# byteowlz/kokorox

Hardware: AMD Instinct MI355X
Metric: real-time factor (audio-s/wall-s), 24 kHz, batch=64 (higher is better)
Workload: dtype f32 in / out, f32 accumulate; products on split operands: f16f8 (a_hi b_hi on f16 MFMAs, the cross terms a_lo b_hi + a_hi b_lo of the 7 / 11-tap convs on e4m3 scaled MFMAs: ~17 significant bits per product; every other conv f16x3: ~22) -- wider than the bf16 BASELINE configs[2] names, inside the 1e-; 1 GPU; batch=64/GPU synthetic 128-phoneme utterances (T=130), durations pinned 3,3,3,4 -> F=422 frames = 10.55 s each, noise on, inputs in HBM; batch_per_gpu=64, frames=422, parallelism=utterance-sharded x1, one-time weight broadcast

## Files before the change

kokorox_amd/build.py:

```python
from __future__ import annotations

import os
import subprocess
import sys

HERE = os.path.dirname(os.path.abspath(__file__))
CSRC = os.path.join(HERE, "csrc")
LIB_DIR = os.path.join(HERE, "lib")
LIB_PATH = os.path.join(LIB_DIR, "libkokorox_hip.so")
TEST_LIB_PATH = os.path.join(LIB_DIR, "libkokorox_hip_test.so")
TEST_SOURCES = ["test_hooks.hip"]
SOURCES = ["conv_plan.hip", "conv_call.hip", "conv_mfma.hip", "conv_f16x3.hip", "conv_f16x3_da.hip", "conv_f16x3_da_p1.hip", "conv_f16x3_da_w2.hip", "conv_f16x3_da_s16.hip", "conv_f16x3_da_f8.hip", "conv_f16x3_da_pre.hip", "conv_f16x3_pre.hip", "conv_f16x3_dapn.hip", "conv_f16x3_dag.hip", "kernels_misc.hip", "model.hip", "model_forward.hip", "model_host.hip", "api.hip", "dispatcher.hip", "onnx_import.cpp", "kxw_file.cpp",
           "host_request.cpp", "host_pool.cpp"]
HEADERS = ["kx_common.h", "kx_error.h", "host_request.h", "conv_epilogue.h", "conv_f16x3_common.h"]
_PUB = os.path.join("..", "..", "include", "kokorox_hip.h")
_PUB_TEST = os.path.join("..", "..", "include", "kokorox_hip_test.h")
_MODEL_H = ["model.h", "kxw_file.h", "onnx_import.h"]
EXTRA_DEPS = {"model.hip": [*_MODEL_H, _PUB], "model_forward.hip": [*_MODEL_H, _PUB], "model_host.hip": [*_MODEL_H, "host_pool.h", _PUB],
              "host_pool.cpp": ["host_pool.h"], "host_request.cpp": ["resample_taps.h"], "kernels_misc.hip": ["resample_taps.h"], "conv_call.hip": _MODEL_H, "api.hip": [*_MODEL_H, "kx_handle.h", "api_guard.h", "check_device.h", _PUB],
              "dispatcher.hip": [*_MODEL_H, "kx_handle.h", "dispatcher_core.h", _PUB],
              "test_hooks.hip": [*_MODEL_H, "kx_handle.h", "api_guard.h", "check_device.h", _PUB, _PUB_TEST], "onnx_import.cpp": ["onnx_import.h"],
              "kxw_file.cpp": ["kxw_file.h", "onnx_import.h"], "conv_f16x3_da_p1.hip": ["conv_f16x3_da.hip"], "conv_f16x3_da_w2.hip": ["conv_f16x3_da.hip"], "conv_f16x3_da_s16.hip": ["conv_f16x3_da.hip"], "conv_f16x3_da_f8.hip": ["conv_f16x3_da.hip"], "conv_f16x3_da_pre.hip": ["conv_f16x3_da.hip"]}
FLAGS = ["-O3", "--offload-arch=gfx950", "-fPIC", "-std=c++17", "-Wall", "-Wno-unused-result"]


def _hipcc() -> str:
    for cand in (os.environ.get("HIPCC"), "/opt/rocm/bin/hipcc", "hipcc"):
        if cand and (os.path.isabs(cand) and os.path.exists(cand) or not os.path.isabs(cand)):
            return cand
    return "hipcc"


def _newer(target: str, deps) -> bool:
    if not os.path.exists(target):
        return False
    t = os.path.getmtime(target)
    return all(os.path.getmtime(d) <= t for d in deps)


LAST_BUILD = {"compiled": [], "reused": [], "linked": False}


def build_library(force: bool = False, verbose: bool = False) -> str:
    LAST_BUILD["compiled"], LAST_BUILD["reused"], LAST_BUILD["linked"] = [], [], False
    os.makedirs(LIB_DIR, exist_ok=True)
# ... 40 lines not shown
```

kokorox_amd/csrc/conv_f16x3.hip:

```cpp
#include "conv_f16x3_common.h"

namespace kx {

template <int BM, int BN, int WM, int WN, int ACT, int TK, bool PF, int VT>
__global__ __launch_bounds__(WM * WN * 64, (WM * WN == 8) ? 4 : ((BM / WM / 32) * (BN / WN / 32) > 6 ? 2 : 3))
void conv1d_f16x3_kernel(const ConvArgs a) {
    constexpr int MT = BM / WM / 32;
    constexpr int NT = BN / WN / 32;
    constexpr int NWV = WM * WN;
    static_assert((NWV == 4 || NWV == 8) && MT >= 1 && NT >= 1, "4 or 8 waves per workgroup");
    static_assert(VT == 1 || (VT <= TK && PF), "virtual taps need TK >= VT and the prefetching build");
    extern __shared__ __attribute__((aligned(16))) unsigned char smem16[];

    const int tid = threadIdx.x;
    const int lane = tid & 63;
    const int wave = __builtin_amdgcn_readfirstlane(tid >> 6);
    const int wm = wave / WN, wn = wave % WN;
    const int r = lane & 31, h = lane >> 5;
    const int b = blockIdx.z, ct = blockIdx.y;
    int tile_x = blockIdx.x;
    if (a.xcd_swizzle && gridDim.x >= 16) {
        const int nx = gridDim.x;
        const int off = (int)(((long)nx * (blockIdx.y + (long)gridDim.y * blockIdx.z)) & 7);
        const int cls = (blockIdx.x + off) & 7;
// ... 364 lines not shown
    else if (bm == 32 && bn == 256 && wm == 1 && wn == 4)
        launch_inst16<32, 256, 1, 4>(p, a, B, s);
    else
        throw Error(1, "conv1d f16x3: no such LDS-DMA form");
}

void launch_conv(const ConvPlan& p, const ConvArgs& a, int B, hipStream_t s) {
    if (p.form == FORM_F32) {
        launch_conv1d(a, p.bm, B, p.cols, s);
        return;
    }
    KX_REQUIRE(a.n_chunks16 == (a.Cin + CK16 - 1) / CK16 && a.w16 != nullptr, "conv1d f16x3: weights not packed");
    KX_REQUIRE(a.epi != EPI_GELU_NEW || p.vt > 1 || p.form == FORM_DAG || p.form == FORM_DAGN,
               "conv1d f16x3: gelu epilogue exists only for k=1 GEMMs with >= 48 input channels");
    KX_REQUIRE(p.merged == (a.merge_T > 0), "conv1d f16x3: merged columns do not match the plan");
    if (p.cols <= 0) return;
    switch (p.form) {
        case FORM_LDS: launch_lds(p, a, B, s); return;
        case FORM_DAG:
        case FORM_DAGN: launch_conv1d_f16x3_dag(p, a, B, s); return;
        case FORM_DAPN: launch_conv1d_f16x3_dapn(a, B, p.cols, s); return;
        case FORM_DA_PRE: launch_conv16_da_pre(p, a, B, s); return;
        case FORM_DA_S16: launch_conv16_da_s16(p, a, B, s); return;
        case FORM_DA_F8: launch_conv16_da_f8(p, a, B, s); return;
        case FORM_DA:
            if (p.p1) {
                launch_conv16_da_p1(p, a, B, s);
                return;
            }
            [[fallthrough]];
        case FORM_DA_W2:
            if (p.form == FORM_DA_W2)
                launch_conv16_da_w2(p, a, B, s);
            else
                launch_conv16_da(p, a, B, s);
            return;
    }
    throw Error(1, "conv1d: unknown kernel form");
}

size_t packed_conv16_halves(int rows, int Cin, int K, int BM) {
    const size_t tiles = (rows + BM - 1) / BM, chunks = (Cin + CK16 - 1) / CK16;
    return tiles * chunks * K * 4 * BM * 8;
}

__global__ void absmax_kernel(const float* p, long n, unsigned* out) {
    float m = 0.f;
// ... 159 lines not shown
```

kokorox_amd/csrc/conv_f16x3_da.hip:

```cpp
#include "conv_f16x3_common.h"
#include <type_traits>


#ifndef KX_F8_RAW_AUX
#define KX_F8_RAW_AUX 0
#endif
#ifndef KX_F8_HWCOS
#define KX_F8_HWCOS 1
#endif

namespace kx {

template <int I, int N, class F>
__device__ __forceinline__ void static_for(F&& f) {
    if constexpr (I < N) {
        f(std::integral_constant<int, I>{});
        static_for<I + 1, N>(f);
    }
}

template <int KT, int RH, int RC, int RAW>
struct F8Sched {
    static constexpr int HS = (KT - 1) / 2, NG = (KT + 1) / 4, NC = 2 * NG;
    static constexpr int cross_of(int p) {
// ... 14 lines not shown
                }
                n += 2;
                st_h[p + RH <= KT - 1 ? sc * KT + p + RH : (sc + 1) * KT + p % RH] = n;
                const int c = cross_of(p);
                if (c >= 0) {
                    n += 4;
                    st_x[sc * NC + c + RC] = n;
                }
            }
            n += RAW;
        }
        return result < 63 ? result : 63;
    }
    static constexpr int cum(int NB, int first, int n) {
        int t = 0;
        for (int r = 0; r < n; ++r) t += cross_of((first + r) / NB) >= 0 ? 3 : 1;
        return t;
    }
    static constexpr int hu_before(int NB, int NA, int HU, int first, int I0, int rel) {
        return rel > I0 ? ((cum(NB, first, rel) - cum(NB, first, I0)) * HU) / (cum(NB, first, NA) - cum(NB, first, I0)) : 0;
    }
};

template <int ACT, int KT, int NTT, bool P1, bool W2 = false, bool S16 = false, bool PRE = false, bool BF = false, bool F8 = false>
__global__ __launch_bounds__(256, (NTT == 8 || S16) ? 2 : 3) void conv1d_f16x3_da_kernel(const ConvArgs a) {
    static_assert(!BF || P1, "BF: a form of the reduced-precision kernels only");
    static_assert(!F8 || (S16 && KT % 4 == 3), "F8: a form of the S16 loop; tap groups of four with one padding slot");
    constexpr bool HWC = F8 && KX_F8_HWCOS;
    static_assert(!PRE || (!P1 && !S16 && ACT == ACT_NONE), "PRE: the activation lives in the image; f16x3 forms on 32x32x16 only");
    static_assert(!W2 || (KT >= 3 && (KT & 1) && NTT == 8), "W2: odd compile-time tap counts on the 256-column tile");
    static_assert(!S16 || (KT >= 3 && (KT & 1) && !P1 && !W2), "S16: odd compile-time tap counts, three MFMAs per product, 4 x 1 waves");
    static_assert(NTT == 8 || NTT == 4 || (NTT == 6 && S16), "tile widths: 256, 128, and 192 columns in the S16 form");
    constexpr int BM = 128, NT = NTT, BN = 32 * NT;
    constexpr bool W64 = KT > 0;
    constexpr bool SPLIT = W64 && BN % 128 == 0;
    constexpr int NJF = W64 ? (SPLIT ? BN / 128 : (BN + 64) / 128) : (BN + 128) / 128;
    constexpr int NJ = NJF + (SPLIT ? 1 : 0);
    constexpr int HU = 8 * NJF + (SPLIT ? 4 : 0);
    constexpr int XWp = W64 ? BN + 64 : BN + 128;
    static_assert(!W64 || SPLIT || (BN + 64) % 128 == 0, "the window is whole 64-column blocks in pairs, or ends in a split block");
    constexpr int XBUF = 4 * XWp;
    constexpr int tap_units = 4 * BM;
    extern __shared__ __attribute__((aligned(16))) unsigned char smem16[];
    uint4* Xs = reinterpret_cast<uint4*>(smem16);

    const int tid = threadIdx.x;
    const int lane = tid & 63;
    const int wave = __builtin_amdgcn_readfirstlane(tid >> 6);
    const int r = lane & 31, h = lane >> 5;
    auto pack_pair = [](float v0, float v1, unsigned& hi_pk, unsigned& lo_pk) __attribute__((always_inline)) {
        if constexpr (BF) {
            auto rne = [](float x) __attribute__((always_inline)) {
                unsigned u = __builtin_bit_cast(unsigned, x);
                u += 0x7fffu + ((u >> 16) & 1u);
                return u >> 16;
            };
            hi_pk = rne(v0) | (rne(v1) << 16);
            lo_pk = 0u;
        } else if constexpr (F8) {
            split_pair_f8(v0, v1, hi_pk, lo_pk);
        } else {
            split_pair(v0, v1, hi_pk, lo_pk);
        }
    };
    auto act_in = [](float y, float slope, float al, float ial) __attribute__((always_inline)) {
        if constexpr (ACT == ACT_SNAKE && HWC) {
            const float u = (al * y) * 0.318309886183790672f;
            return __builtin_fmaf(ial, __builtin_fmaf(-0.5f, __builtin_amdgcn_cosf(u), 0.5f), y);
        } else {
            return in_act<ACT>(y, slope, al, ial);
        }
// ... 30 lines not shown
        if (a.xcd_swizzle && N >= 16) {
            const int off = (int)(((long)N * blockIdx.z) & 7);
            const int cls = (l + off) & 7;
            int start = 0;
            for (int c = 0; c < cls; ++c) {
                const int first = (c - off) & 7;
                start += first < N ? (N - first + 7) >> 3 : 0;
            }
            lp = start + (l >> 3);
        }
        if (a.xcd_swizzle) {
            tile_x = lp / ny;
            ct = lp - tile_x * ny;
        }
    }
    if (a.dephase_cycles > 0) {
        const unsigned gl = blockIdx.x + gridDim.x * (blockIdx.y + gridDim.y * blockIdx.z);
        const bool late = a.dephase_mode == 1 ? (gl < 512u && ((gl >> 3) & 1u)) : (gl >= 256u && gl < 512u);
        if (late) {
            const unsigned long long t_end = __builtin_amdgcn_s_memtime() + (unsigned long long)a.dephase_cycles;
            while (__builtin_amdgcn_s_memtime() < t_end) __builtin_amdgcn_s_sleep(64);
        }
    }
    const int t0 = tile_x * BN;
    const int Lin = a.in_len.lens[b] * a.in_len.mul + a.in_len.add;
    const int Lout = a.out_len.lens[b] * a.out_len.mul + a.out_len.add;
    const int ncols = (a.store == ST_UPSCATTER) ? (Lin + 1) : Lout;
    if (t0 >= ncols) return;

    const int K = KT > 0 ? KT : a.K, dil = a.dil;
    const int n_chunks = a.n_chunks16;
    const int n_steps = n_chunks * K;
    const float* xb = a.x + (long)b * a.x_bs;
    const int p0 = t0 - a.pad;
    const bool has_norm = a.nmean != nullptr;
    const int up2 = a.in_up2;
    const int Lsrc = up2 ? ((Lin + 1) >> 1) : Lin;

    f32x16 acc[1][NT];
#pragma unroll
    for (int j = 0; j < NT; ++j)
#pragma unroll
        for (int e = 0; e < 16; ++e) acc[0][j][e] = 0.f;
    constexpr int NB16 = S16 ? 2 * NT : 1;
    f32x4v acc16[2][NB16];
#pragma unroll
    for (int i = 0; i < 2; ++i)
#pragma unroll
        for (int j = 0; j < NB16; ++j) acc16[i][j] = f32x4v{0.f, 0.f, 0.f, 0.f};

    const int g = wave & 1, jb = wave >> 1;
    float raw[NJ][8];
    float praw[4];
    int xoff[NJ];
    unsigned okmask = 0;
    auto blk_col = [&](int j) __attribute__((always_inline)) { return (SPLIT && j == NJF) ? 64 * 2 * NJF : 64 * (jb + 2 * j); };
#pragma unroll
    for (int j = 0; j < NJ; ++j) {
        const int p = p0 + lane + blk_col(j);
        okmask |= (p >= 0 && p < Lin) ? (1u << j) : 0u;
        int pi = up2 ? (p >> 1) : p;
        pi = pi < 0 ? 0 : (pi >= Lsrc ? Lsrc - 1 : pi);
        xoff[j] = pi;
    }
    using u32x4 = __attribute__((ext_vector_type(4))) unsigned;
    constexpr int NLD = PRE ? (4 * XWp) / 256 : 1;
    static_assert(!PRE || (4 * XWp) % 256 == 0, "PRE: whole rounds of 256 lanes");
    u32x4 rawq[NLD];
    unsigned qoff[NLD];
    unsigned okq = 0;
    const buf_rsrc xq = make_buf(PRE ? reinterpret_cast<const char*>(a.x16) + (long)b * a.x16_bs : reinterpret_cast<const char*>(a.x));
    const unsigned chunk_bytes = PRE ? 64u * (unsigned)a.x16_ld : 0u;
    const buf_rsrc xrow = make_buf(xb);
    if constexpr (PRE) {
#pragma unroll
        for (int i = 0; i < NLD; ++i) {
            const int idx = tid + 256 * i, plane = idx / XWp, u = idx - plane * XWp;
            const int p = p0 + u;
            okq |= (p >= 0 && p < Lin) ? (1u << i) : 0u;
// ... 282 lines not shown
#define KX_F8_RC (NT == 6 ? 1 : 2)
#endif
        constexpr int RH = KX_F8_RH, RC = KX_F8_RC;
        using FS = F8Sched<KT, RH, RC, raw_ops>;
        constexpr int NG = FS::NG, NC = FS::NC;
        static_assert(RH <= KT && (KT - 1) % RH != 0 && NC % RC == 0, "f16f8: static ring slots");
        static_assert(2 * (NG - 1) <= HS && KT - 1 - 2 * (NG - 1) >= HS && (HS & 1), "f16f8: cross groups inside their buffer's phase");
        const int n_super = n_chunks >> 1;
        const int d_norm = tau16 ? dil : 0, d_str = tau16 ? XBUF - (KT - 1) * dil : 0;
        int d_x2 = tau16 ? 2 * dil : 0;
        int d_xl = tau16 ? 0 : dil;
        using v8i = __attribute__((ext_vector_type(8))) int;
        u32x4 hs[RH][2], xs[RC][4];
        auto make_srd = [](const void* base) __attribute__((always_inline)) {
            const unsigned long long pa = (unsigned long long)base;
            u32x4 srd;
            srd[0] = __builtin_amdgcn_readfirstlane((unsigned)pa);
            srd[1] = __builtin_amdgcn_readfirstlane((unsigned)(pa >> 32) & 0xffffu);
            srd[2] = 0xffffffffu;
            srd[3] = 0x00020000u;
            return srd;
        };
        const u32x4 srd_h = make_srd(a.w16), srd_x = make_srd(a.w8x);
        const unsigned voff_h = 16u * (unsigned)(tau16 * tap_units + h16 * BM + wave * 32 + r16);
        const unsigned voff_x = 16u * (unsigned)((lane >> 4) * 256 + wave * 32 + r16);
        const unsigned tile_h = (unsigned)__builtin_amdgcn_readfirstlane(ct * n_steps), tile_x8 = (unsigned)__builtin_amdgcn_readfirstlane(ct * n_chunks * NG);
        auto load_H = [&](int s0, u32x4 (&xh)[2]) __attribute__((always_inline)) {
            const unsigned so = (tile_h + (unsigned)__builtin_amdgcn_readfirstlane(s0 < n_steps - 2 ? s0 : n_steps - 2)) * (16u * tap_units);
            asm volatile("buffer_load_dwordx4 %0, %1, %2, %3 offen" : "=v"(xh[0]) : "v"(voff_h), "s"(srd_h), "s"(so) : "memory");
            asm volatile("buffer_load_dwordx4 %0, %1, %2, %3 offen offset:256" : "=v"(xh[1]) : "v"(voff_h), "s"(srd_h), "s"(so) : "memory");
        };
        auto load_X = [&](int chunk, const int m, u32x4 (&x)[4]) __attribute__((always_inline)) {
            const unsigned so = (tile_x8 + (unsigned)__builtin_amdgcn_readfirstlane(chunk < n_chunks ? chunk : n_chunks - 1) * NG + m) * 16384u;
            asm volatile("buffer_load_dwordx4 %0, %1, %2, %3 offen" : "=v"(x[0]) : "v"(voff_x), "s"(srd_x), "s"(so) : "memory");
            asm volatile("buffer_load_dwordx4 %0, %1, %2, %3 offen offset:2048" : "=v"(x[1]) : "v"(voff_x), "s"(srd_x), "s"(so) : "memory");
            asm volatile("buffer_load_dwordx4 %0, %1, %2, %3 offen offset:256" : "=v"(x[2]) : "v"(voff_x), "s"(srd_x), "s"(so) : "memory");
            asm volatile("buffer_load_dwordx4 %0, %1, %2, %3 offen offset:2304" : "=v"(x[3]) : "v"(voff_x), "s"(srd_x), "s"(so) : "memory");
        };
        static_for<0, RH>([&](auto qc) __attribute__((always_inline)) { load_H(2 * decltype(qc)::value, hs[decltype(qc)::value]); });
        static_for<0, RC>([&](auto qc) __attribute__((always_inline)) {
            constexpr int c = decltype(qc)::value;
            load_X(c >= NG ? 1 : 0, c >= NG ? c - NG : c, xs[c]);
        });
        asm volatile("s_waitcnt vmcnt(0)" ::: "memory");
        int xl_it = h16 * XWp + r16;
        int dil_it = dil;
        half8 fh[2];
        v8i fx[2];
        auto load_blk_h = [&](const int p, const int nb, half8& fhx) __attribute__((always_inline)) {
// ... 533 lines not shown
                    age += raw_ops;
                    o1 += raw_ops;
                    o2 += raw_ops;
                }
                load_tile(0, 0, fh[(E0 + NT) % 3], fl[(E0 + NT) % 3]);
                load_tile(0, 1, fh[(E0 + NT + 1) % 3], fl[(E0 + NT + 1) % 3]);
            }
        }
    };
    for (int s3 = 0; s3 < n_steps; s3 += 3) {
        step(0, ah0, al0, age0, age1, age2, s3);
        if (s3 + 1 < n_steps) step(NT % 3, ah1, al1, age1, age2, age0, s3 + 1);
        if (s3 + 2 < n_steps) step((2 * NT) % 3, ah2, al2, age2, age0, age1, s3 + 2);
    }
    }
    asm volatile("s_waitcnt vmcnt(0)" ::: "memory");
    if (a.dbg & 8) return;
    asm volatile("s_waitcnt lgkmcnt(0)\n\ts_barrier" ::: "memory");
    float2* stat_scr = reinterpret_cast<float2*>(smem16) + wave * (32 * 33);
    float* wide_scr = reinterpret_cast<float*>(stat_scr);
    if constexpr (S16) {
        static_for<0, NT / 2>([&](auto gc) __attribute__((always_inline)) {
            constexpr int g2 = decltype(gc)::value;
            conv_store_group16<EPI_ROWS, NB16, 2, NT == 6>(a, acc16, 4 * g2, a.w_unscale, b, ct * BM + wave * 32, t0 + 64 * g2, lane, ncols, Lout,
                                                  tile_x * (NT / 2) + g2, stat_scr, wide_scr);
        });
    } else if constexpr (W2) {
        conv_store_group<EPI_ROWS, true>(a, *reinterpret_cast<f32x16(*)[1][4]>(&acc[0][0]), a.w_unscale, b, ct * BM + wr2 * 64, t0 + 128 * wc2, r,
                                   h, ncols, Lout, tile_x * 2 + wc2, stat_scr, wide_scr);
        conv_store_group<EPI_ROWS, true>(a, *reinterpret_cast<f32x16(*)[1][4]>(&acc[0][4]), a.w_unscale, b, ct * BM + wr2 * 64 + 32, t0 + 128 * wc2,
                                   r, h, ncols, Lout, tile_x * 2 + wc2, stat_scr, wide_scr);
    } else if constexpr (NT == 8) {
        conv_store_group<EPI_ROWS>(a, *reinterpret_cast<f32x16(*)[1][4]>(&acc[0][0]), a.w_unscale, b, ct * BM + wave * 32, t0, r, h,
                                   ncols, Lout, tile_x * 2, stat_scr, wide_scr);
        conv_store_group<EPI_ROWS>(a, *reinterpret_cast<f32x16(*)[1][4]>(&acc[0][4]), a.w_unscale, b, ct * BM + wave * 32, t0 + 128, r,
                                   h, ncols, Lout, tile_x * 2 + 1, stat_scr, wide_scr);
    } else {
        conv_store_group<EPI_ROWS>(a, acc, a.w_unscale, b, ct * BM + wave * 32, t0, r, h, ncols, Lout, tile_x, stat_scr, wide_scr);
    }
}

template <int ACT, int KT, int NTT, bool P1 = false, bool W2 = false, bool S16 = false, bool PRE = false, bool BF = false, bool F8 = false>
static void launch_da_inst(const ConvArgs& a, int B, int max_cols, hipStream_t s) {
    auto kern = conv1d_f16x3_da_kernel<ACT, KT, NTT, P1, W2, S16, PRE, BF, F8>;
    constexpr int BN = 32 * NTT;
    constexpr size_t lds_x = 16 * (size_t)2 * 4 * (BN + 128), lds_scr = 4 * 32 * 33 * sizeof(float2);
    constexpr size_t lds = lds_x > lds_scr ? lds_x : lds_scr;
    KX_REQUIRE(a.stride == 1 && a.merge_T == 0 && (a.K - 1) * a.dil + 256 <= 384, "conv1d f16x3 da: launch not eligible");
    dim3 grid((max_cols + BN - 1) / BN, (a.Cout + 127) / 128, B);
    KX_REQUIRE(grid.x > 0 && grid.y > 0 && grid.y < 65536 && B > 0 && B < 65536, "conv1d f16x3 da: bad grid");
    if (a.tile_prefix) {
        KX_REQUIRE(a.flat_ny == (int)grid.y && a.flat_B == B && a.flat_bn_host == BN && a.flat_tiles_host > 0 &&
                       (long)a.flat_tiles_host * grid.y < (1L << 30),
                   "conv1d f16x3 da: flat tile list does not match the launch");
        grid = dim3((unsigned)a.flat_tiles_host * grid.y, 1, 1);
    }
    hipLaunchKernelGGL(kern, grid, dim3(256), lds, s, a);
    KX_HIP(hipGetLastError());
}

template <int NTT, bool P1, bool BF>
static void launch_da_4x1(const ConvPlan& p, const ConvArgs& a, int B, hipStream_t s) {
#ifdef KX_DA_AUDIT
    if (p.act == ACT_SNAKE) launch_da_inst<ACT_SNAKE, 11, 8, P1, false, false, false, BF>(a, B, p.cols, s);
    else launch_da_inst<ACT_LEAKY, 0, 4, P1, false, false, false, BF>(a, B, p.cols, s);
    return;
#endif
    KX_REQUIRE(p.kt == 0 || (a.K == p.kt && (a.K - 1) * a.dil <= 64), "conv1d f16x3 da: compile-time taps do not match the launch");
    if (p.act == ACT_SNAKE) {
        if (p.kt == 11) launch_da_inst<ACT_SNAKE, 11, NTT, P1, false, false, false, BF>(a, B, p.cols, s);
        else if (p.kt == 7) launch_da_inst<ACT_SNAKE, 7, NTT, P1, false, false, false, BF>(a, B, p.cols, s);
        else if (p.kt == 3) launch_da_inst<ACT_SNAKE, 3, NTT, P1, false, false, false, BF>(a, B, p.cols, s);
        else launch_da_inst<ACT_SNAKE, 0, NTT, P1, false, false, false, BF>(a, B, p.cols, s);
    } else if (p.act == ACT_LEAKY) {
        if (p.kt == 3) launch_da_inst<ACT_LEAKY, 3, NTT, P1, false, false, false, BF>(a, B, p.cols, s);
        else launch_da_inst<ACT_LEAKY, 0, NTT, P1, false, false, false, BF>(a, B, p.cols, s);
    } else
        launch_da_inst<ACT_NONE, 0, NTT, P1, false, false, false, BF>(a, B, p.cols, s);
}

template <bool P1, bool BF>
static void launch_da_4x1_bn(const ConvPlan& p, const ConvArgs& a, int B, hipStream_t s) {
    KX_REQUIRE(p.bn == 256 || p.bn == 128, "conv1d f16x3 da: tile of 256 or 128 columns");
// ... 13 lines not shown
```

kokorox_amd/csrc/conv_plan.hip:

```cpp
#include "kx_common.h"

namespace kx {

static bool da_eligible(int BM, int K, int dil, int stride, bool merged) {
    return BM == 128 && stride == 1 && !merged && (K - 1) * dil + 256 <= 384;
}

static bool f8_taps(int K, int dil) { return (K == 11 || K == 7 || K == 3) && (K - 1) * dil <= 64; }

static bool s16_shape(int BM, int K, int dil, int stride, int act, int n_chunks16, bool merged, int pmode) {
    const bool taps = K == 11 || (K == 7 && dil == 1) || (pmode == 2 && f8_taps(K, dil));
    return BM == 128 && stride == 1 && !merged && pmode != 1 && act == ACT_SNAKE && taps && (K - 1) * dil <= 64 && n_chunks16 >= 2 &&
           (n_chunks16 & 1) == 0;
}

bool conv16_f8_layer(int BM, int rows, int K, int n_chunks16) {
    return BM == 128 && f8_taps(K, 1) && (K != 3 || rows <= 256) && n_chunks16 >= 2 && (n_chunks16 & 1) == 0;
}

ConvPlan conv_plan(const ConvLaunch& c) {
    ConvPlan p{};
    p.bm = c.BM;
    p.act = c.act;
    p.vt = 1;
    p.cols = c.cols;
    const bool stats = c.stats && c.store == ST_NORMAL && !c.accum;
    auto set_stats = [&](int stat_cols) {
        if (!stats) return;
        p.stat_cols = stat_cols;
        p.stat_tiles = (p.cols + p.bn - 1) / p.bn * (p.bn / stat_cols);
    };
    if (c.mode == CONV_F32) {
        p.form = FORM_F32;
        p.bn = c.BM == 128 ? 128 : 256;
        set_stats(64);
        return p;
    }
// ... 22 lines not shown
        const long tiles = (long)((p.cols + 127) / 128) * ((c.rows + 127) / 128);
        if (route != FORCE_LDS && !c.norm && c.store != ST_UPSCATTER) {
            const long wgs = tiles * (p.merged ? 1 : c.B);
            const bool narrow_ok = (c.x_bs * c.B + 16L * c.x_ld) * 4 < (1L << 31);
            p.form = narrow_ok && 2 * wgs <= c.cus ? FORM_DAGN : FORM_DAG;
            p.bn = p.form == FORM_DAGN ? 32 : 128;
            return p;
        }
        p.form = FORM_LDS;
        p.bn = 128;
        p.wm = 2;
        p.wn = 2;
        p.pf = 1;
        p.vt = tiles > 2L * c.cus ? 2 : 3;
        return p;
    }

    const bool da = route != FORCE_LDS && da_eligible(c.BM, c.K, c.dil, c.stride, p.merged);
    const bool small = (long)((p.cols + 255) / 256) * ((c.rows + 127) / 128) * c.B < 256;
    if (route != FORCE_LDS && !(c.force & FORCE_NO_S16) && s16_shape(c.BM, c.K, c.dil, c.stride, c.act, c.n_chunks16, p.merged, pmode)) {
        p.form = pmode == 2 ? FORM_DA_F8 : FORM_DA_S16;
        p.kt = c.K;
        p.bn = small && route != FORCE_DA ? 128 : 192;
        set_stats(64);
    } else if (!da || (route != FORCE_DA && c.cols <= 160 && !stats)) {
        p.form = FORM_LDS;
        const bool short_seq = c.cols <= 160 && !stats;
        p.bn = !short_seq && !small ? 256 : 128;
        p.wm = !short_seq && small ? 4 : 2;
        p.wn = !short_seq && small ? 1 : 2;
        p.pf = c.stride == 1 && (c.K - 1) * c.dil <= 128;
        set_stats(p.bn / p.wn);
    } else {
        p.bn = small && route != FORCE_DA ? 128 : 256;
        set_stats(128);
        const bool w64 = (c.K - 1) * c.dil <= 64;
        if (p.pre) {
            const bool narrow = p.bn == 128 && !c.prec1 && c.rows % 32 == 0 && c.K <= 12 && c.epi == EPI_NONE &&
                                (c.store == ST_NORMAL || c.store == ST_UPSCATTER) && (long)c.n_chunks16 * c.K < 5000;
            p.form = narrow ? FORM_DAPN : FORM_DA_PRE;
            p.act = ACT_NONE;
            p.kt = c.K == 3 && w64 ? 3 : 0;
        } else {
            const bool unrolled = w64 && ((c.act == ACT_SNAKE && (c.K == 11 || c.K == 7 || c.K == 3)) || (c.act == ACT_LEAKY && c.K == 3));
            p.kt = unrolled ? c.K : 0;
            p.p1 = c.prec1 != 0;
// ... 11 lines not shown
```

kokorox_amd/csrc/kx_common.h:

```cpp
#pragma once
#include <hip/hip_runtime.h>

#include <cmath>
#include <cstdint>
#include <cstring>
#include <cstdio>
#include <stdexcept>
#include <string>
#include <vector>

#include <atomic>
#include <mutex>

#include "host_request.h"
#include "kx_error.h"

namespace kx {

constexpr int KX_MAX_DEVICES = 64;

struct DynLdsLimit {
    std::atomic<size_t> limit[KX_MAX_DEVICES];
    std::mutex mu;
    DynLdsLimit() {
// ... 81 lines not shown
    int dbg;
    const int* tile_prefix;
    int flat_ny;
    int flat_B;
    int flat_tiles_host, flat_bn_host;
    const void* x16;
    long x16_bs;
    int x16_ld;
};

enum ConvMode { CONV_F32 = 0, CONV_F16X3 = 1, CONV_F16X3_LDS = 2, CONV_F16X3_DA = 3, CONV_F16 = 4, CONV_BF16 = 5, CONV_F16F8 = 6 };
enum ConvForm {
    FORM_F32 = 0,
    FORM_LDS,
    FORM_DAG,
    FORM_DAGN,
    FORM_DA,
    FORM_DA_W2,
    FORM_DA_S16,
    FORM_DA_F8,
    FORM_DA_PRE,
    FORM_DAPN,
};
enum ConvForce { FORCE_LDS = 1, FORCE_DA = 2, FORCE_DA_4X1 = 4, FORCE_NO_S16 = 8 };

struct ConvLaunch {
    int mode;
    int prec1;
    int f8;
    int BM, rows, n_chunks16, K, dil, stride, pad, act, in_up2, store, accum, epi;
    int norm;
    int stats;
    int image;
    int merge_T;
    long x_bs;
    int x_ld;
    int B, cols;
    int cus;
    int force;
};
struct ConvPlan {
    int form;
    int bm, act, kt, wm, wn, vt, pf, p1, bf;
    int bn;
    int cols;
    int merged;
    int pre;
    int stat_cols, stat_tiles;
    int flat_bn;
};
ConvPlan conv_plan(const ConvLaunch& c);
bool conv16_f8_layer(int BM, int rows, int K, int n_chunks16);
void launch_conv(const ConvPlan& p, const ConvArgs& a, int B, hipStream_t s);
int conv16_cu_count();
int cu_count_override();

size_t conv16_pre_image_bytes(int Cin, int x_ld);
void launch_split_image(const ConvArgs& a, int B, int Lmax, void* img, long img_bs, hipStream_t s);

void launch_tile_prefix(LenMap len, int extra, int bn, int B, int* out, hipStream_t s);

inline int conv_pick_bm(int rows) { return rows >= 128 ? 128 : (rows > 32 ? 64 : 32); }

void launch_conv1d(const ConvArgs& a, int BM, int B, int max_cols, hipStream_t s);

struct PackSrc {
    const float* p[3];
    int rows[3];
};
void launch_pack_conv(const PackSrc& src, float* dst, int Cout, int Cin, int K, int BM, hipStream_t s);
void launch_pack_convT(const float* w, float* dst, int Cin, int Cout, int s, int BM, hipStream_t s_);
size_t packed_conv_floats(int rows, int Cin, int K, int BM);

void launch_conv16_da(const ConvPlan& p, const ConvArgs& a, int B, hipStream_t s);
void launch_conv16_da_p1(const ConvPlan& p, const ConvArgs& a, int B, hipStream_t s);
void launch_conv16_da_w2(const ConvPlan& p, const ConvArgs& a, int B, hipStream_t s);
void launch_conv16_da_s16(const ConvPlan& p, const ConvArgs& a, int B, hipStream_t s);
void launch_conv16_da_f8(const ConvPlan& p, const ConvArgs& a, int B, hipStream_t s);
void launch_conv16_da_pre(const ConvPlan& p, const ConvArgs& a, int B, hipStream_t s);
void launch_conv1d_f16x3_dapn(const ConvArgs& a, int B, int max_cols, hipStream_t s);
void launch_conv1d_f16x3_dag(const ConvPlan& p, const ConvArgs& a, int B, hipStream_t s);
size_t packed_conv16_halves(int rows, int Cin, int K, int BM);
float device_absmax(const float* p, long n, hipStream_t s);
int pick_weight_shift(float absmax);
void launch_pack_conv16(const PackSrc& src, void* dst, int Cout, int Cin, int K, int BM, float wscale, hipStream_t s);
void launch_pack_convT16(const float* w, void* dst, int Cin, int Cout, int sd, int BM, float wscale, hipStream_t s);
void launch_image_to_bf16(const void* w16, void* dst, size_t n_halves, hipStream_t s);
size_t packed_conv8x_bytes(int rows, int Cin, int K);
void launch_pack_conv8x(const void* w16, void* dst, int rows, int Cin, int K, hipStream_t s);

void launch_vec_add(const float* a, const float* b, float* out, int n, hipStream_t s);
void launch_transpose_whh(const float* whh, float* out, hipStream_t s);

void launch_albert_embed(const int64_t* ids, long ids_stride, const float* word, const float* type0,
                         const float* pos, float* out, long bs, int ld, const int* lens, int B, int Tmax,
                         int n_vocab, unsigned* bad_id, hipStream_t s);
void launch_embed(const int64_t* ids, long ids_stride, const float* table, int C, float* out, long bs, int ld,
                  const int* lens, int B, int Tmax, int n_vocab, unsigned* bad_id, hipStream_t s);

enum LnMode { LN_PLAIN = 0, LN_AFFINE = 1, LN_ADA = 2 };
void launch_layernorm_ch(const float* x, float* y, long bs, int ld, int C, LenMap len, int B, int Lmax,
// ... 71 lines not shown
```

kokorox_amd/csrc/model.h:

```cpp
#pragma once
#include <atomic>
#include <chrono>
#include <functional>
#include <map>
#include <mutex>
#include <string>
#include <vector>

#include "kx_common.h"
#include "kxw_file.h"

namespace kx {

struct ConvW {
    const float* w = nullptr;
    const float* bias = nullptr;
    int rows = 0, Cin = 0, K = 0, BM = 0, n_chunks = 0;
    int up_s = 0, up_cout = 0;
    const void* w16 = nullptr;
    const void* w16b = nullptr;
    const void* w8x = nullptr;
    int n_chunks16 = 0;
    float unscale = 1.f;
    std::string name;
// ... 78 lines not shown
    int n_bs = 0;
    int force = 0;
    int image = 0;
    int epi_stream = -1;
    bool offer_merge = true;
    bool flat = true;
    bool stats = false;
};

struct ConvCall {
    ConvPlan plan;
    ConvArgs a;
    int B;
    size_t image_bytes() const { return conv16_pre_image_bytes(a.Cin, a.x_ld); }
    void set_image(const void* img, long img_bs) {
        a.x16 = img;
        a.x16_bs = img_bs;
        a.x16_ld = a.x_ld;
    }
    const LenMap& flat_len() const { return a.store == ST_UPSCATTER ? a.in_len : a.out_len; }
    int flat_extra() const { return a.store == ST_UPSCATTER ? 1 : 0; }
    void set_flat(const int* tile_prefix, int tiles_host) {
        a.tile_prefix = tile_prefix;
        a.flat_ny = (a.Cout + 127) / 128;
        a.flat_B = B;
        a.flat_tiles_host = tiles_host;
        a.flat_bn_host = plan.flat_bn;
    }
    void set_stats(float2* part) {
        a.stat_part = part;
        a.stat_tiles = plan.stat_tiles;
    }
};
ConvCall conv_call(const ConvW& w, const T& in, const T& out, const ConvOpts& o, const ConvCtx& ctx);
int conv_tile_count(const int* h_lens, int B, const LenMap& lm, int extra, int bn);

struct LstmTimeout : Error {
    explicit LstmTimeout(const std::string& m) : Error(3, m) {}
};

template <class V>
struct Restore {
    V& ref;
    V saved;
    Restore(V& r, V now) : ref(r), saved(r) { ref = now; }
    ~Restore() { ref = saved; }
    Restore(const Restore&) = delete;
// ... 223 lines not shown
```

kokorox_amd/hip_koko.py:

```python
from __future__ import annotations

import ctypes as C
import os
from typing import List, Optional, Sequence

import numpy as np

_HERE = os.path.dirname(os.path.abspath(__file__))
LIB_PATH = os.path.join(_HERE, "lib", "libkokorox_hip.so")

PACK_F32_MONO, PACK_F32_STEREO, PACK_PCM16_MONO = 0, 1, 2
PACK_WAV_F32, PACK_WAV16_BASE64 = 3, 4
PACK_MULAW, PACK_ALAW = 8, 9
PACK_RATE_24000, PACK_RATE_8000, PACK_RATE_16000, PACK_RATE_48000 = 0x000, 0x100, 0x200, 0x300
RATE_HZ = {0: 24000, 1: 8000, 2: 16000, 3: 48000}
RESAMPLE_MAX_TAPS = 145
KX_OK, KX_ERR_INVALID, KX_ERR_IO, KX_ERR_DEVICE, KX_ERR_STATE = 0, 1, 2, 3, 4
KX_FLAG_NOISE_OFF = 1
KX_FLAG_TAPS = 2
STYLE_DIM = 256
SAMPLES_PER_FRAME = 600

_lib = None

# ... 664 lines not shown
           device=0, mode=None, pre=False):
    lib = load_test_library()
    if mode is None:
        mode = CONV_F32 if os.environ.get("KOKOROX_CONV", "") == "f32" else CONV_F16X3
    x, w = _f32(x), _f32(w)
    B, Cin, L = x.shape
    k = w.shape[2]
    if transposed:
        Cout = w.shape[1]
        Lout = (L - 1) * stride - 2 * pad + k
    else:
        Cout = w.shape[0]
        Lout = (L + 2 * pad - dil * (k - 1) - 1) // stride + 1
    y = np.zeros((B, Cout, Lout), dtype=np.float32)
    bias, alpha, norm = _f32(bias), _f32(alpha), _f32(norm)
    _err_call(lib.kx_test_conv1d, device, _ptr(x), B, Cin, L, _ptr(w), _ptr(bias), Cout, k, stride, pad, dil,
              1 if transposed else 0, act, float(slope), _ptr(alpha), _ptr(norm), _ptr(y), Lout, mode | (0x100 if pre else 0))
    return y


CONV_LAUNCH_FIELDS = ("mode", "prec1", "f8", "BM", "rows", "n_chunks16", "K", "dil", "stride", "pad", "act", "in_up2", "store", "accum",
                      "epi", "norm", "stats", "image", "merge_T", "x_bs", "x_ld", "B", "cols", "cus", "force")
CONV_PLAN_FIELDS = ("form", "bm", "act", "kt", "wm", "wn", "vt", "pf", "p1", "bf", "bn", "cols", "merged", "pre", "stat_cols",
                    "stat_tiles", "flat_bn")
CONV_FORMS = ("F32", "LDS", "DAG", "DAGN", "DA", "DA_W2", "DA_S16", "DA_F8", "DA_PRE", "DAPN")


def conv_plan(**launch):
    lib = load_test_library()
    unknown = set(launch) - set(CONV_LAUNCH_FIELDS)
    assert not unknown, unknown
    src = np.array([int(launch.get(f, 0)) for f in CONV_LAUNCH_FIELDS], dtype=np.int64)
    out = np.zeros(len(CONV_PLAN_FIELDS), dtype=np.int64)
    _err_call(lib.kx_test_conv_plan, _ptr(src), len(src), _ptr(out), len(out))
    plan = dict(zip(CONV_PLAN_FIELDS, (int(v) for v in out)))
    plan["form"] = CONV_FORMS[plan["form"]]
    return plan


def conv_transpose(x, w, bias=None, stride=6, act=1, slope=0.1, resid=None, up_off=0, mode=1, pre=False, device=0):
    lib = load_test_library()
    x, w = _f32(x), _f32(w)
    B, Cin, L = x.shape
    Cout, k = w.shape[1], w.shape[2]
    assert k == 2 * stride
    pad = (k - stride) // 2
    Lout = (L - 1) * stride - 2 * pad + k
# ... 169 lines not shown
```

Measured before the change: 6845 x realtime.

## Add 256-row, 8-wave variant of f16f8 direct conv kernel sharing input tile

Adds a 512-thread form of the f16f8 direct-access conv kernel. Two groups of four waves cover two adjacent 128-row output-channel tiles over the same 192-column input window, so the staged input in LDS is shared across 256 output rows. The planner picks it for f8 snake convs with rows divisible by 256, for k=3 taps or dilated k=7 taps, and the flat tile grid is sized to match. This halves the input staging and LDS traffic per output row, at the cost of one workgroup per CU (launch bounds 512,1) and fewer tiles in the grid, which may lower occupancy and load balance.

```diff
diff --git a/kokorox_amd/build.py b/kokorox_amd/build.py
--- a/kokorox_amd/build.py
+++ b/kokorox_amd/build.py
@@ -10,7 +10,7 @@
 LIB_PATH = os.path.join(LIB_DIR, "libkokorox_hip.so")
 TEST_LIB_PATH = os.path.join(LIB_DIR, "libkokorox_hip_test.so")
 TEST_SOURCES = ["test_hooks.hip"]
-SOURCES = ["conv_plan.hip", "conv_call.hip", "conv_mfma.hip", "conv_f16x3.hip", "conv_f16x3_da.hip", "conv_f16x3_da_p1.hip", "conv_f16x3_da_w2.hip", "conv_f16x3_da_s16.hip", "conv_f16x3_da_f8.hip", "conv_f16x3_da_pre.hip", "conv_f16x3_pre.hip", "conv_f16x3_dapn.hip", "conv_f16x3_dag.hip", "kernels_misc.hip", "model.hip", "model_forward.hip", "model_host.hip", "api.hip", "dispatcher.hip", "onnx_import.cpp", "kxw_file.cpp",
+SOURCES = ["conv_plan.hip", "conv_call.hip", "conv_mfma.hip", "conv_f16x3.hip", "conv_f16x3_da.hip", "conv_f16x3_da_p1.hip", "conv_f16x3_da_w2.hip", "conv_f16x3_da_s16.hip", "conv_f16x3_da_f8.hip", "conv_f16x3_da_f8w.hip", "conv_f16x3_da_pre.hip", "conv_f16x3_pre.hip", "conv_f16x3_dapn.hip", "conv_f16x3_dag.hip", "kernels_misc.hip", "model.hip", "model_forward.hip", "model_host.hip", "api.hip", "dispatcher.hip", "onnx_import.cpp", "kxw_file.cpp",
            "host_request.cpp", "host_pool.cpp"]
 HEADERS = ["kx_common.h", "kx_error.h", "host_request.h", "conv_epilogue.h", "conv_f16x3_common.h"]
 _PUB = os.path.join("..", "..", "include", "kokorox_hip.h")
@@ -20,7 +20,7 @@
               "host_pool.cpp": ["host_pool.h"], "host_request.cpp": ["resample_taps.h"], "kernels_misc.hip": ["resample_taps.h"], "conv_call.hip": _MODEL_H, "api.hip": [*_MODEL_H, "kx_handle.h", "api_guard.h", "check_device.h", _PUB],
               "dispatcher.hip": [*_MODEL_H, "kx_handle.h", "dispatcher_core.h", _PUB],
               "test_hooks.hip": [*_MODEL_H, "kx_handle.h", "api_guard.h", "check_device.h", _PUB, _PUB_TEST], "onnx_import.cpp": ["onnx_import.h"],
-              "kxw_file.cpp": ["kxw_file.h", "onnx_import.h"], "conv_f16x3_da_p1.hip": ["conv_f16x3_da.hip"], "conv_f16x3_da_w2.hip": ["conv_f16x3_da.hip"], "conv_f16x3_da_s16.hip": ["conv_f16x3_da.hip"], "conv_f16x3_da_f8.hip": ["conv_f16x3_da.hip"], "conv_f16x3_da_pre.hip": ["conv_f16x3_da.hip"]}
+              "kxw_file.cpp": ["kxw_file.h", "onnx_import.h"], "conv_f16x3_da_p1.hip": ["conv_f16x3_da.hip"], "conv_f16x3_da_w2.hip": ["conv_f16x3_da.hip"], "conv_f16x3_da_s16.hip": ["conv_f16x3_da.hip"], "conv_f16x3_da_f8.hip": ["conv_f16x3_da.hip"], "conv_f16x3_da_f8w.hip": ["conv_f16x3_da.hip"], "conv_f16x3_da_pre.hip": ["conv_f16x3_da.hip"]}
 FLAGS = ["-O3", "--offload-arch=gfx950", "-fPIC", "-std=c++17", "-Wall", "-Wno-unused-result"]
 
 
diff --git a/kokorox_amd/csrc/conv_f16x3.hip b/kokorox_amd/csrc/conv_f16x3.hip
--- a/kokorox_amd/csrc/conv_f16x3.hip
+++ b/kokorox_amd/csrc/conv_f16x3.hip
@@ -410,7 +410,10 @@
         case FORM_DAPN: launch_conv1d_f16x3_dapn(a, B, p.cols, s); return;
         case FORM_DA_PRE: launch_conv16_da_pre(p, a, B, s); return;
         case FORM_DA_S16: launch_conv16_da_s16(p, a, B, s); return;
-        case FORM_DA_F8: launch_conv16_da_f8(p, a, B, s); return;
+        case FORM_DA_F8:
+            if (p.rows256) launch_conv16_da_f8w(p, a, B, s);
+            else launch_conv16_da_f8(p, a, B, s);
+            return;
         case FORM_DA:
             if (p.p1) {
                 launch_conv16_da_p1(p, a, B, s);
diff --git a/kokorox_amd/csrc/conv_f16x3_da.hip b/kokorox_amd/csrc/conv_f16x3_da.hip
--- a/kokorox_amd/csrc/conv_f16x3_da.hip
+++ b/kokorox_amd/csrc/conv_f16x3_da.hip
@@ -60,19 +60,25 @@
     }
 };
 
+constexpr int NTT_ROWS256 = 16;
+
 template <int ACT, int KT, int NTT, bool P1, bool W2 = false, bool S16 = false, bool PRE = false, bool BF = false, bool F8 = false>
-__global__ __launch_bounds__(256, (NTT == 8 || S16) ? 2 : 3) void conv1d_f16x3_da_kernel(const ConvArgs a) {
+__global__ __launch_bounds__(NTT >= NTT_ROWS256 ? 512 : 256, NTT >= NTT_ROWS256 ? 1 : ((NTT == 8 || S16) ? 2 : 3)) void conv1d_f16x3_da_kernel(const ConvArgs a) {
+    constexpr bool R8 = NTT >= NTT_ROWS256;
+    constexpr int NTC = R8 ? NTT - NTT_ROWS256 : NTT;
+    static_assert(!R8 || (F8 && NTC == 6), "R8: a form of the f16f8 loop on the 192-column tile");
     static_assert(!BF || P1, "BF: a form of the reduced-precision kernels only");
     static_assert(!F8 || (S16 && KT % 4 == 3), "F8: a form of the S16 loop; tap groups of four with one padding slot");
     constexpr bool HWC = F8 && KX_F8_HWCOS;
     static_assert(!PRE || (!P1 && !S16 && ACT == ACT_NONE), "PRE: the activation lives in the image; f16x3 forms on 32x32x16 only");
-    static_assert(!W2 || (KT >= 3 && (KT & 1) && NTT == 8), "W2: odd compile-time tap counts on the 256-column tile");
+    static_assert(!W2 || (KT >= 3 && (KT & 1) && NTC == 8), "W2: odd compile-time tap counts on the 256-column tile");
     static_assert(!S16 || (KT >= 3 && (KT & 1) && !P1 && !W2), "S16: odd compile-time tap counts, three MFMAs per product, 4 x 1 waves");
-    static_assert(NTT == 8 || NTT == 4 || (NTT == 6 && S16), "tile widths: 256, 128, and 192 columns in the S16 form");
-    constexpr int BM = 128, NT = NTT, BN = 32 * NT;
+    static_assert(NTC == 8 || NTC == 4 || (NTC == 6 && S16), "tile widths: 256, 128, and 192 columns in the S16 form");
+    constexpr int BM = 128, NT = NTC, BN = 32 * NT;
     constexpr bool W64 = KT > 0;
     constexpr bool SPLIT = W64 && BN % 128 == 0;
-    constexpr int NJF = W64 ? (SPLIT ? BN / 128 : (BN + 64) / 128) : (BN + 128) / 128;
+    constexpr int NWP = R8 ? 4 : 2;
+    constexpr int NJF = W64 ? (SPLIT ? BN / 128 : (BN + 64) / (64 * NWP)) : (BN + 128) / 128;
     constexpr int NJ = NJF + (SPLIT ? 1 : 0);
     constexpr int HU = 8 * NJF + (SPLIT ? 4 : 0);
     constexpr int XWp = W64 ? BN + 64 : BN + 128;
@@ -85,6 +91,7 @@
     const int tid = threadIdx.x;
     const int lane = tid & 63;
     const int wave = __builtin_amdgcn_readfirstlane(tid >> 6);
+    const int wrow = R8 ? (wave & 3) : wave;
     const int r = lane & 31, h = lane >> 5;
     auto pack_pair = [](float v0, float v1, unsigned& hi_pk, unsigned& lo_pk) __attribute__((always_inline)) {
         if constexpr (BF) {
@@ -161,6 +168,7 @@
             while (__builtin_amdgcn_s_memtime() < t_end) __builtin_amdgcn_s_sleep(64);
         }
     }
+    const int ctw = R8 ? 2 * ct + (wave >> 2) : ct;
     const int t0 = tile_x * BN;
     const int Lin = a.in_len.lens[b] * a.in_len.mul + a.in_len.add;
     const int Lout = a.out_len.lens[b] * a.out_len.mul + a.out_len.add;
@@ -193,7 +201,7 @@
     float praw[4];
     int xoff[NJ];
     unsigned okmask = 0;
-    auto blk_col = [&](int j) __attribute__((always_inline)) { return (SPLIT && j == NJF) ? 64 * 2 * NJF : 64 * (jb + 2 * j); };
+    auto blk_col = [&](int j) __attribute__((always_inline)) { return (SPLIT && j == NJF) ? 64 * 2 * NJF : 64 * (jb + NWP * j); };
 #pragma unroll
     for (int j = 0; j < NJ; ++j) {
         const int p = p0 + lane + blk_col(j);
@@ -522,9 +530,9 @@
             return srd;
         };
         const u32x4 srd_h = make_srd(a.w16), srd_x = make_srd(a.w8x);
-        const unsigned voff_h = 16u * (unsigned)(tau16 * tap_units + h16 * BM + wave * 32 + r16);
-        const unsigned voff_x = 16u * (unsigned)((lane >> 4) * 256 + wave * 32 + r16);
-        const unsigned tile_h = (unsigned)__builtin_amdgcn_readfirstlane(ct * n_steps), tile_x8 = (unsigned)__builtin_amdgcn_readfirstlane(ct * n_chunks * NG);
+        const unsigned voff_h = 16u * (unsigned)(tau16 * tap_units + h16 * BM + wrow * 32 + r16);
+        const unsigned voff_x = 16u * (unsigned)((lane >> 4) * 256 + wrow * 32 + r16);
+        const unsigned tile_h = (unsigned)__builtin_amdgcn_readfirstlane(ctw * n_steps), tile_x8 = (unsigned)__builtin_amdgcn_readfirstlane(ctw * n_chunks * NG);
         auto load_H = [&](int s0, u32x4 (&xh)[2]) __attribute__((always_inline)) {
             const unsigned so = (tile_h + (unsigned)__builtin_amdgcn_readfirstlane(s0 < n_steps - 2 ? s0 : n_steps - 2)) * (16u * tap_units);
             asm volatile("buffer_load_dwordx4 %0, %1, %2, %3 offen" : "=v"(xh[0]) : "v"(voff_h), "s"(srd_h), "s"(so) : "memory");
@@ -1104,7 +1112,7 @@
     if constexpr (S16) {
         static_for<0, NT / 2>([&](auto gc) __attribute__((always_inline)) {
             constexpr int g2 = decltype(gc)::value;
-            conv_store_group16<EPI_ROWS, NB16, 2, NT == 6>(a, acc16, 4 * g2, a.w_unscale, b, ct * BM + wave * 32, t0 + 64 * g2, lane, ncols, Lout,
+            conv_store_group16<EPI_ROWS, NB16, 2, NT == 6>(a, acc16, 4 * g2, a.w_unscale, b, ctw * BM + wrow * 32, t0 + 64 * g2, lane, ncols, Lout,
                                                   tile_x * (NT / 2) + g2, stat_scr, wide_scr);
         });
     } else if constexpr (W2) {
@@ -1141,6 +1149,27 @@
     KX_HIP(hipGetLastError());
 }
 
+template <int KT>
+static void launch_da_rows256(const ConvArgs& a, int B, int max_cols, hipStream_t s) {
+    auto kern = conv1d_f16x3_da_kernel<ACT_SNAKE, KT, 6 + NTT_ROWS256, false, false, true, false, false, true>;
+    constexpr int BN = 192;
+    constexpr size_t lds_x = 16 * (size_t)2 * 4 * (BN + 64), lds_scr = 8 * 32 * 33 * sizeof(float2);
+    constexpr size_t lds = lds_x > lds_scr ? lds_x : lds_scr;
+    KX_REQUIRE(a.stride == 1 && a.merge_T == 0 && (a.K - 1) * a.dil <= 64 && a.Cout % 256 == 0, "conv1d f16x3 da rows256: launch not eligible");
+    dim3 grid((max_cols + BN - 1) / BN, a.Cout / 256, B);
+    KX_REQUIRE(grid.x > 0 && grid.y > 0 && grid.y < 65536 && B > 0 && B < 65536, "conv1d f16x3 da rows256: bad grid");
+    if (a.tile_prefix) {
+        KX_REQUIRE(a.flat_ny == (int)grid.y && a.flat_B == B && a.flat_bn_host == BN && a.flat_tiles_host > 0 &&
+                       (long)a.flat_tiles_host * grid.y < (1L << 30),
+                   "conv1d f16x3 da rows256: flat tile list does not match the launch");
+        grid = dim3((unsigned)a.flat_tiles_host * grid.y, 1, 1);
+    }
+    static DynLdsLimit lds_limit;
+    lds_limit.ensure(reinterpret_cast<const void*>(kern), lds);
+    hipLaunchKernelGGL(kern, grid, dim3(512), lds, s, a);
+    KX_HIP(hipGetLastError());
+}
+
 template <int NTT, bool P1, bool BF>
 static void launch_da_4x1(const ConvPlan& p, const ConvArgs& a, int B, hipStream_t s) {
 #ifdef KX_DA_AUDIT
diff --git a/kokorox_amd/csrc/conv_f16x3_da_f8w.hip b/kokorox_amd/csrc/conv_f16x3_da_f8w.hip
--- /dev/null
+++ b/kokorox_amd/csrc/conv_f16x3_da_f8w.hip
@@ -0,0 +1,25 @@
+#define KX_DA_UNIT
+#ifndef KX_F8_I0A_LONG
+#define KX_F8_I0A_LONG 40
+#endif
+#ifndef KX_F8_I0A_MID
+#define KX_F8_I0A_MID 16
+#endif
+#ifndef KX_F8_I0B
+#define KX_F8_I0B 8
+#endif
+#include "conv_f16x3_da.hip"
+
+namespace kx {
+
+void launch_conv16_da_f8w(const ConvPlan& p, const ConvArgs& a, int B, hipStream_t s) {
+    KX_REQUIRE(p.form == FORM_DA_F8 && p.rows256 && p.bn == 192 && a.w8x != nullptr && (p.kt == 11 || p.kt == 7 || p.kt == 3) && a.K == p.kt &&
+                   (a.K - 1) * a.dil <= 64 && a.act == ACT_SNAKE && !a.prec1 && a.n_chunks16 >= 2 && (a.n_chunks16 & 1) == 0 && a.Cout % 256 == 0,
+               "conv1d f16x3 da f8 rows256: launch not eligible");
+    KX_REQUIRE((long)a.Cin * a.x_ld * 4 < (1L << 32), "conv1d f16x3 da f8 rows256: input tensor of one utterance beyond 4 GiB");
+    if (p.kt == 11) launch_da_rows256<11>(a, B, p.cols, s);
+    else if (p.kt == 7) launch_da_rows256<7>(a, B, p.cols, s);
+    else launch_da_rows256<3>(a, B, p.cols, s);
+}
+
+}
diff --git a/kokorox_amd/csrc/conv_plan.hip b/kokorox_amd/csrc/conv_plan.hip
--- a/kokorox_amd/csrc/conv_plan.hip
+++ b/kokorox_amd/csrc/conv_plan.hip
@@ -13,6 +13,8 @@
     return BM == 128 && stride == 1 && !merged && pmode != 1 && act == ACT_SNAKE && taps && (K - 1) * dil <= 64 && n_chunks16 >= 2 &&
            (n_chunks16 & 1) == 0;
 }
+
+static bool rows256_taps(int K, int dil) { return K == 3 || (K == 7 && dil > 1); }
 
 bool conv16_f8_layer(int BM, int rows, int K, int n_chunks16) {
     return BM == 128 && f8_taps(K, 1) && (K != 3 || rows <= 256) && n_chunks16 >= 2 && (n_chunks16 & 1) == 0;
@@ -81,6 +83,8 @@
         p.form = pmode == 2 ? FORM_DA_F8 : FORM_DA_S16;
         p.kt = c.K;
         p.bn = small && route != FORCE_DA ? 128 : 192;
+        p.rows256 = p.form == FORM_DA_F8 && p.bn == 192 && c.rows % 256 == 0 && !(c.force & FORCE_ROWS128) &&
+                    (route == FORCE_DA || rows256_taps(c.K, c.dil));
         set_stats(64);
     } else if (!da || (route != FORCE_DA && c.cols <= 160 && !stats)) {
         p.form = FORM_LDS;
diff --git a/kokorox_amd/csrc/kx_common.h b/kokorox_amd/csrc/kx_common.h
--- a/kokorox_amd/csrc/kx_common.h
+++ b/kokorox_amd/csrc/kx_common.h
@@ -127,7 +127,7 @@
     FORM_DA_PRE,
     FORM_DAPN,
 };
-enum ConvForce { FORCE_LDS = 1, FORCE_DA = 2, FORCE_DA_4X1 = 4, FORCE_NO_S16 = 8 };
+enum ConvForce { FORCE_LDS = 1, FORCE_DA = 2, FORCE_DA_4X1 = 4, FORCE_NO_S16 = 8, FORCE_ROWS128 = 16 };
 
 struct ConvLaunch {
     int mode;
@@ -153,6 +153,7 @@
     int pre;
     int stat_cols, stat_tiles;
     int flat_bn;
+    int rows256;
 };
 ConvPlan conv_plan(const ConvLaunch& c);
 bool conv16_f8_layer(int BM, int rows, int K, int n_chunks16);
@@ -182,6 +183,7 @@
 void launch_conv16_da_w2(const ConvPlan& p, const ConvArgs& a, int B, hipStream_t s);
 void launch_conv16_da_s16(const ConvPlan& p, const ConvArgs& a, int B, hipStream_t s);
 void launch_conv16_da_f8(const ConvPlan& p, const ConvArgs& a, int B, hipStream_t s);
+void launch_conv16_da_f8w(const ConvPlan& p, const ConvArgs& a, int B, hipStream_t s);
 void launch_conv16_da_pre(const ConvPlan& p, const ConvArgs& a, int B, hipStream_t s);
 void launch_conv1d_f16x3_dapn(const ConvArgs& a, int B, int max_cols, hipStream_t s);
 void launch_conv1d_f16x3_dag(const ConvPlan& p, const ConvArgs& a, int B, hipStream_t s);
diff --git a/kokorox_amd/csrc/model.h b/kokorox_amd/csrc/model.h
--- a/kokorox_amd/csrc/model.h
+++ b/kokorox_amd/csrc/model.h
@@ -124,7 +124,7 @@
     int flat_extra() const { return a.store == ST_UPSCATTER ? 1 : 0; }
     void set_flat(const int* tile_prefix, int tiles_host) {
         a.tile_prefix = tile_prefix;
-        a.flat_ny = (a.Cout + 127) / 128;
+        a.flat_ny = plan.rows256 ? a.Cout / 256 : (a.Cout + 127) / 128;
         a.flat_B = B;
         a.flat_tiles_host = tiles_host;
         a.flat_bn_host = plan.flat_bn;
diff --git a/kokorox_amd/hip_koko.py b/kokorox_amd/hip_koko.py
--- a/kokorox_amd/hip_koko.py
+++ b/kokorox_amd/hip_koko.py
@@ -710,7 +710,7 @@
 CONV_LAUNCH_FIELDS = ("mode", "prec1", "f8", "BM", "rows", "n_chunks16", "K", "dil", "stride", "pad", "act", "in_up2", "store", "accum",
                       "epi", "norm", "stats", "image", "merge_T", "x_bs", "x_ld", "B", "cols", "cus", "force")
 CONV_PLAN_FIELDS = ("form", "bm", "act", "kt", "wm", "wn", "vt", "pf", "p1", "bf", "bn", "cols", "merged", "pre", "stat_cols",
-                    "stat_tiles", "flat_bn")
+                    "stat_tiles", "flat_bn", "rows256")
 CONV_FORMS = ("F32", "LDS", "DAG", "DAGN", "DA", "DA_W2", "DA_S16", "DA_F8", "DA_PRE", "DAPN")
 
 
```

Result: no change. 6882 x realtime (median of 6 runs) (+0.5%).
